# CEA-LIST/runia_core

Measured on AMD Instinct MI355X. Metric: OOD scores/sec, LaREM 16-MC PCA-256 (ResNet-18 layer4 latent 512x4x4), higher is better.
Workload: dtype f64

## Files before the change

### include/runia_hip.h

```cpp
#ifndef RUNIA_HIP_H
#define RUNIA_HIP_H

#include <stddef.h>
#include <stdint.h>

#ifdef __cplusplus
extern "C" {
#endif

#define RUNIA_OK 0
#define RUNIA_E_INVALID (-1)
#define RUNIA_E_LAUNCH (-2)
#define RUNIA_E_NODEVICE (-3)
#define RUNIA_E_WORKSPACE (-4)

typedef void* runia_stream_t;

int runia_abi_version(void);
const char* runia_error_string(int code);
int runia_device_count(void);
int runia_clock_probe(uint64_t* out4, int chain, runia_stream_t stream);
int runia_time_next_launch(void* start_event, void* stop_event);

int runia_mc_stack_f32(const float* x, const float* rand, int64_t rand_image_stride, float* out,
// ... 110 lines not shown
int runia_mc_entropy_f32(const float* x, const float* rand, int64_t rand_image_stride, double* h,
                         float* z_out, double* zero_fill, void* workspace, size_t workspace_bytes, int64_t N,
                         int C, int H, int W, int n_mc, double drop_prob, int block_size, int k, double min_dist,
                         runia_stream_t stream);
int runia_mc_draws_f32(float* out, int64_t N, int n_mc, int H, int W, uint64_t seed, int64_t first_image,
                       runia_stream_t stream);
int runia_mc_mask_table_counter_f32(uint64_t seed, int64_t first_image, void* workspace, size_t workspace_bytes,
                                    int64_t N, int H, int W, int n_mc, double drop_prob, int block_size,
                                    int redraw_dead_layers, runia_stream_t stream);
int runia_mc_entropy_counter_f32(const float* x, uint64_t seed, int64_t first_image, double* h, float* z_out,
                                 double* zero_fill, void* workspace, size_t workspace_bytes, int64_t N, int C, int H,
                                 int W, int n_mc, double drop_prob, int block_size, int k, double min_dist,
                                 int redraw_dead_layers, runia_stream_t stream);
int runia_pca_md_score_f64(const double* h, const double* packed_ct, const double* bias,
                           const double* scale, const double* md_mean, const double* packed_p,
                           double* score, double* y_out, int64_t N, int64_t D, int64_t n,
                           runia_stream_t stream);
size_t runia_proj_sq_workspace_bytes(int64_t N);
int runia_proj_sq_accumulate_f64(const double* h, const double* packed_m, const double* c, double* score,
                                 int64_t N, int64_t D, int64_t r, runia_stream_t stream);
int runia_proj_sq_score_f64(const double* h, const double* packed_m, const double* c, double* score,
                            void* workspace, size_t workspace_bytes, int64_t N, int64_t D, int64_t r,
                            runia_stream_t stream);

size_t runia_covariance_workspace_bytes(int64_t N, int64_t D);
int runia_covariance_f64(const double* x, double* mean, double* cov, void* workspace,
                         size_t workspace_bytes, int64_t N, int64_t D, runia_stream_t stream);
int runia_covariance_f32in(const float* x, double* mean, double* cov, void* workspace,
                           size_t workspace_bytes, int64_t N, int64_t D, runia_stream_t stream);

int runia_roi_align_f32(const float* input, const float* boxes, const int* batch_idx, float* out, int64_t K, int64_t B,
                        int C, int H, int W, int PH, int PW, double spatial_scale, int sampling_ratio, int aligned,
                        runia_stream_t stream);
int runia_nchw_to_nhwc_f32(const float* in, float* out, int64_t B, int C, int64_t HW, runia_stream_t stream);
int runia_roi_mc_entropy_supported(int PH, int PW, int n_mc, int k, int sampling_ratio);
size_t runia_roi_mc_entropy_workspace_bytes(int64_t K, int PH, int PW, int n_mc, int sampling_ratio);
int runia_roi_mc_entropy_f32(const float* feat_nhwc, const float* boxes, const int* batch_idx, const float* rand,
                             int64_t rand_image_stride, double* h, float* z_out, void* workspace, size_t workspace_bytes,
                             int64_t K, int64_t B, int C, int H, int W, int PH, int PW, double spatial_scale,
                             int sampling_ratio, int aligned, int n_mc, double drop_prob, int block_size, int k,
                             double min_dist, runia_stream_t stream);
#define RUNIA_ROI_MEANS_MAX_HW 2048
int runia_roi_means_f32(const float* feat_nhwc, const float* boxes, const int* batch_idx, float* out, int64_t ldo,
                        int64_t col_offset, int64_t K, int64_t B, int C, int H, int W, int PH, int PW, double spatial_scale,
                        int sampling_ratio, int aligned, runia_stream_t stream);

// ... 183 lines not shown
```

### runia_core_amd/_hip.py

```python
from __future__ import annotations

import contextlib
import ctypes
import os
import threading
from ctypes import c_char_p, c_double, c_float, c_int, c_int64, c_size_t, c_uint64, c_void_p
from typing import NamedTuple, Optional, Union

import numpy as np
import torch

from . import config as _config

_LIB_PATH = os.path.join(os.path.dirname(os.path.abspath(__file__)), "librunia_hip.so")
_lib: Optional[ctypes.CDLL] = None

_SIGNATURES = {
    "runia_abi_version": (c_int, []),
    "runia_error_string": (c_char_p, [c_int]),
    "runia_device_count": (c_int, []),
    "runia_clock_probe": (c_int, [c_void_p, c_int, c_void_p]),
    "runia_time_next_launch": (c_int, [c_void_p, c_void_p]),
    "runia_mc_stack_f32": (
        c_int,
        [c_void_p, c_void_p, c_int64, c_void_p, c_int64, c_int, c_int, c_int, c_int, c_double, c_int, c_void_p],
    ),
    "runia_mc_drop_flat_f32": (
        c_int,
        [c_void_p, c_void_p, c_int64, c_void_p, c_int64, c_int, c_int, c_int, c_int, c_double, c_int, c_void_p],
    ),
# ... 132 lines not shown
    "runia_roi_mc_entropy_supported": (c_int, [c_int, c_int, c_int, c_int, c_int]),
    "runia_roi_mc_entropy_workspace_bytes": (c_size_t, [c_int64, c_int, c_int, c_int, c_int]),
    "runia_roi_mc_entropy_f32": (
        c_int,
        [c_void_p, c_void_p, c_void_p, c_void_p, c_int64, c_void_p, c_void_p, c_void_p, c_size_t, c_int64, c_int64, c_int, c_int,
         c_int, c_int, c_int, c_double, c_int, c_int, c_int, c_double, c_int, c_int, c_double, c_void_p],
    ),
    "runia_roi_means_f32": (
        c_int,
        [c_void_p, c_void_p, c_void_p, c_void_p, c_int64, c_int64, c_int64, c_int64, c_int, c_int, c_int, c_int, c_int,
         c_double, c_int, c_int, c_void_p],
    ),
    "runia_linear_f32": (c_int, [c_void_p, c_void_p, c_void_p, c_void_p, c_int64, c_int64, c_int64, c_float, c_void_p]),
    "runia_ash_s_f32": (c_int, [c_void_p, c_void_p, c_int64, c_int64, c_int, c_void_p]),
    "runia_gen_score_f32": (c_int, [c_void_p, c_void_p, c_int64, c_int64, c_int, c_double, c_void_p]),
    "runia_gen_entropy_f32": (c_int, [c_void_p, c_void_p, c_int64, c_int64, c_int, c_double, c_void_p]),
    "runia_mcd_uncertainty_f32": (c_int, [c_void_p, c_void_p, c_void_p, c_void_p, c_int64, c_int, c_int64, c_void_p]),
    "runia_ash_s_rows_f32": (c_int, [c_void_p, c_void_p, c_void_p, c_int64, c_int64, c_int, c_int, c_void_p]),
    "runia_tril_inverse_f64": (c_int, [c_void_p, c_void_p, c_int64, c_int64, c_void_p]),
    "runia_proj_norm_f32": (c_int, [c_void_p, c_void_p, c_void_p, c_void_p, c_int64, c_int64, c_int64, c_void_p]),
    "runia_proj_norm_f64": (c_int, [c_void_p, c_void_p, c_void_p, c_void_p, c_int64, c_int64, c_int64, c_void_p]),
    "runia_proj_sq_workspace_bytes": (c_size_t, [c_int64]),
    "runia_proj_sq_accumulate_f64": (c_int, [c_void_p, c_void_p, c_void_p, c_void_p, c_int64, c_int64, c_int64, c_void_p]),
    "runia_proj_sq_score_f64": (
        c_int,
        [c_void_p, c_void_p, c_void_p, c_void_p, c_void_p, c_size_t, c_int64, c_int64, c_int64, c_void_p],
    ),
    "runia_covariance_workspace_bytes": (c_size_t, [c_int64, c_int64]),
    "runia_covariance_f64": (c_int, [c_void_p, c_void_p, c_void_p, c_void_p, c_size_t, c_int64, c_int64, c_void_p]),
    "runia_covariance_f32in": (c_int, [c_void_p, c_void_p, c_void_p, c_void_p, c_size_t, c_int64, c_int64, c_void_p]),
    "runia_rauq_workspace_bytes": (c_size_t, [c_int64, c_int64, c_int64, c_int64, c_int64, c_int]),
    "runia_rauq_gather": (c_int, [c_void_p, c_int, c_int64, c_int64, c_int64, c_int, c_void_p, c_void_p]),
    "runia_rauq_score": (
        c_int,
        [c_void_p, c_int64, c_int64, c_int64, c_int, c_void_p, c_void_p, c_int, c_void_p, c_void_p, c_void_p, c_size_t, c_void_p],
    ),
    "runia_rauq_rollout_rows": (
        c_int, [c_void_p, c_int, c_int64, c_int64, c_int64, c_int64, c_void_p, c_void_p, c_size_t, c_void_p]),
    "runia_rauq_rollout_att": (
        c_int,
        [c_void_p, c_int, c_int64, c_int64, c_int64, c_int64, c_int, c_int, c_int64, c_void_p, c_void_p, c_size_t, c_void_p],
    ),
    "runia_rauqb_workspace_bytes": (c_size_t, [c_int64, c_int64, c_int64, c_int64, c_int64, c_int]),
    "runia_rauqb_gather": (c_int, [c_void_p, c_void_p, c_int, c_int64, c_int64, c_int64, c_int64, c_int, c_void_p, c_void_p]),
    "runia_rauqb_score": (
        c_int,
        [c_void_p, c_void_p, c_int64, c_int64, c_int64, c_int64, c_int, c_int, c_void_p, c_int64, c_void_p, c_int, c_void_p,
# ... 918 lines not shown
        xp, hp = x.data_ptr() + done * c * hh * ww * 4, h.data_ptr() + done * c * 8
        rp = None if rand is None else rand.data_ptr() + done * stride * 4
        zp = None if z is None else z.data_ptr() + done * n_mc * c * 4
        zf = None if zero_fill is None else zero_fill.data_ptr() + done * 8
        if kernel_events is not None:
            if counter is not None:
                launch("runia_mc_mask_table_counter_f32", seed, int(counter.first_image) + done, ws.data_ptr(), ws_bytes, m, hh,
                       ww, n_mc, float(drop_prob), int(block_size), redraw)
            else:
                launch("runia_mc_mask_table_f32", rp, stride, ws.data_ptr(), ws_bytes, m, hh, ww, n_mc, float(drop_prob),
                       int(block_size))
            kernel_events.append(_timed_call("runia_mc_entropy_from_table_f32", xp, ws.data_ptr(), ws_bytes, hp, zp, zf, m, c, hh,
                                             ww, n_mc, int(k), float(min_dist)))
        elif counter is not None:
            launch("runia_mc_entropy_counter_f32", xp, seed, int(counter.first_image) + done, hp, zp, zf, ws.data_ptr(), ws_bytes,
                   m, c, hh, ww, n_mc, float(drop_prob), int(block_size), int(k), float(min_dist), redraw)
        else:
            launch("runia_mc_entropy_f32", xp, rp, stride, hp, zp, zf, ws.data_ptr(), ws_bytes, m, c, hh, ww, n_mc,
                   float(drop_prob), int(block_size), int(k), float(min_dist))
    return (h, z) if want_samples else h


@_device_guard()
def proj_sq_accumulate(h: torch.Tensor, packed_m: torch.Tensor, c: torch.Tensor, r: int, out: torch.Tensor) -> torch.Tensor:
    require_gpu()
    assert h.is_cuda and h.dtype == torch.float64 and h.dim() == 2
    h = h.contiguous()
    nrow, d = h.shape
    assert out.is_cuda and out.dtype == torch.float64 and out.shape == (nrow,) and out.is_contiguous()
    launch("runia_proj_sq_accumulate_f64", h.data_ptr(), packed_m.data_ptr(), c.data_ptr(), out.data_ptr(), nrow, d, int(r))
    return out


@_device_guard()
def pca_md_score(h: torch.Tensor, packed_ct: Optional[torch.Tensor], bias: Optional[torch.Tensor],
                 scale: Optional[torch.Tensor], md_mean: torch.Tensor, packed_p: torch.Tensor, n: int,
                 want_projection: bool = False, out: Optional[torch.Tensor] = None):
    require_gpu()
    assert h.is_cuda and h.dtype == torch.float64 and h.dim() == 2
    h = h.contiguous()
    nrow, d = h.shape
    if out is None:
        s = torch.empty((nrow,), dtype=torch.float64, device=h.device)
    else:
        assert out.is_cuda and out.dtype == torch.float64 and out.shape == (nrow,) and out.is_contiguous()
        s = out
    y = torch.empty((nrow, n), dtype=torch.float64, device=h.device) if want_projection else None
    launch("runia_pca_md_score_f64", h.data_ptr(), _ptr(packed_ct), _ptr(bias), _ptr(scale), md_mean.data_ptr(),
           packed_p.data_ptr(), s.data_ptr(), _ptr(y), nrow, d, n)
    return (s, y) if want_projection else s


@_device_guard()
# ... 133 lines not shown
@_device_guard()
def gen_score(logits: torch.Tensor, gamma: float, m: int) -> torch.Tensor:
    require_gpu()
    assert logits.is_cuda and logits.dtype == torch.float32 and logits.dim() == 2
    logits = logits.contiguous()
    s = torch.empty((logits.shape[0],), dtype=torch.float32, device=logits.device)
    launch("runia_gen_score_f32", logits.data_ptr(), s.data_ptr(), logits.shape[0], logits.shape[1], int(m), float(gamma))
    return s


@_device_guard()
def proj_norm(x: torch.Tensor, u: torch.Tensor, packed_ns: torch.Tensor, n: int) -> torch.Tensor:
    require_gpu()
    assert x.is_cuda and x.dim() == 2 and x.dtype == u.dtype and x.dtype in (torch.float32, torch.float64)
    x, u = x.contiguous(), u.contiguous()
    nrow, d = x.shape
    out = torch.empty((nrow,), dtype=torch.float64, device=x.device)
    launch("runia_proj_norm_f32" if x.dtype == torch.float32 else "runia_proj_norm_f64", x.data_ptr(), u.data_ptr(),
           packed_ns.data_ptr(), out.data_ptr(), nrow, d, int(n))
    return out


@_device_guard()
def proj_sq_score(h: torch.Tensor, packed_m: torch.Tensor, c: torch.Tensor, r: int, out: Optional[torch.Tensor] = None) -> torch.Tensor:
    lib = load_library()
    require_gpu()
    assert h.is_cuda and h.dtype == torch.float64 and h.dim() == 2
    h = h.contiguous()
    nrow, d = h.shape
    s = torch.empty((nrow,), dtype=torch.float64, device=h.device) if out is None else out
    ws_bytes = int(lib.runia_proj_sq_workspace_bytes(nrow))
    ws = torch.empty(max(ws_bytes, 16), dtype=torch.uint8, device=h.device)
    launch("runia_proj_sq_score_f64", h.data_ptr(), packed_m.data_ptr(), c.data_ptr(), s.data_ptr(), ws.data_ptr(), ws_bytes,
           nrow, d, int(r))
    return s


def _ood_metrics_buffers(n: int, device):
    ws_bytes = query("runia_ood_metrics_workspace_bytes", n)
    ws = workspace(ws_bytes + 256, device, 0)
    return ws, ws.data_ptr() + (-ws.data_ptr()) % 256, ws_bytes, torch.empty(3, dtype=torch.float64, device=device)


@_device_guard()
def ood_metrics(ind_scores: torch.Tensor, ood_scores: torch.Tensor) -> torch.Tensor:
    require_gpu()
    assert ind_scores.is_cuda and ood_scores.is_cuda and ind_scores.dtype == ood_scores.dtype
    assert ind_scores.dtype in (torch.float32, torch.float64)
    a, b = ind_scores.reshape(-1).contiguous(), ood_scores.reshape(-1).contiguous()
    n = a.numel() + b.numel()
    ws, ws_ptr, ws_bytes, out = _ood_metrics_buffers(n, a.device)
    launch("runia_ood_metrics_f64" if a.dtype == torch.float64 else "runia_ood_metrics_f32", a.data_ptr(), a.numel(),
           b.data_ptr(), b.numel(), out.data_ptr(), ws_ptr, ws_bytes)
    return out


@_device_guard()
def ood_clf_curve(ind_scores: torch.Tensor, ood_scores: torch.Tensor):
# ... 443 lines not shown
```

### runia_core_amd/csrc/fused.hip

```cpp
#include "common.hpp"
#include "entropy_core.hpp"
#include "mfma_f64_tile.hpp"
#include "philox.hpp"
#include "div_consts.hpp"

namespace {

using namespace runia_entropy;
using namespace runia_mfma;

constexpr int kMaxMC = 64;
typedef float f2 __attribute__((ext_vector_type(2)));

__device__ __forceinline__ void layer_consts(int cnt, int& m, float& flag, float& zh, float& zl) {
  const int a = cnt ? __ffs(cnt) - 1 : 0;
  m = cnt >> a;
  flag = __uint_as_float((unsigned)(127 - a) << 23);
  zh = cnt ? __uint_as_float(runia_div::kDivHi[(m - 1) >> 1]) : NAN;
  zl = cnt ? __uint_as_float(runia_div::kDivLo[(m - 1) >> 1]) : 0.f;
}

__device__ __forceinline__ float add_f32(float a, float b) {
  float r;
  asm("v_add_f32 %0, %1, %2" : "=v"(r) : "v"(a), "v"(b));
// ... 531 lines not shown
    const int64_t row = r0 + tid;
    if (row < g.N) g.score[row] = -(((part[tid] + part[BM + tid]) + part[2 * BM + tid]) + part[3 * BM + tid]);
  }
}

struct ProjSqArgs {
  const double* h;
  const double* packed_m;
  const double* c;
  double* score;
  double* partial;
  int64_t N, D, r;
};

#ifndef K2_WAVES
#define K2_WAVES 5
#endif
#ifndef K2_DMA
#define K2_DMA 1
#endif
#ifndef K2_WAVES_DMA
#define K2_WAVES_DMA 5
#endif
template <int RT, int NCT, bool ACCUMULATE, bool SPLIT, bool DMA>
__global__ __launch_bounds__(256, (RT == 1 && NCT <= 2) ? (DMA ? K2_WAVES_DMA : K2_WAVES) : 1) void proj_sq_kernel(ProjSqArgs g) {
#if defined(__HIP_DEVICE_COMPILE__)
  constexpr int BM = 16 * RT;
  __shared__ double lds_a[DMA ? 1 : 2 * BM * APITCH];
  __shared__ __attribute__((aligned(16))) double lds_d0[DMA ? BM * KC : 2];
  __shared__ __attribute__((aligned(16))) double lds_d1[DMA ? BM * KC : 2];
  constexpr int NG = (NCT + 1) / 2;
  __shared__ double part[4 * NG * BM];
  const int64_t n_pad = n_padded(g.r);
  const int tid = threadIdx.x, lane = tid & 63;
  const int wave = __builtin_amdgcn_readfirstlane(tid >> 6);
  const int li = lane & 15, lg = lane >> 4;
  const int64_t NT = n_pad / 16;
  int64_t tile = blockIdx.x;
  int half = 0;
  if constexpr (SPLIT) {
    tile = (int64_t)(blockIdx.x >> 4) * 8 + (blockIdx.x & 7);
    half = (blockIdx.x >> 3) & 1;
    if (tile * BM >= g.N) return;
  }
  const int64_t r0 = tile * BM;
  const int nchunks = (int)(k_padded(g.D) / KC);
  constexpr int PER_T = BM * KC / 256;
  double rowsq[NG][RT][4];
#pragma unroll
  for (int q = 0; q < NG; ++q)
#pragma unroll
    for (int a = 0; a < RT; ++a)
#pragma unroll
      for (int r = 0; r < 4; ++r) rowsq[q][a][r] = 0.0;
  for (int64_t cb = 0; cb < n_pad / BN; ++cb) {
    const int64_t ctbase = cb * 16 + (int64_t)half * (4 * NCT) + wave * NCT;
    d4 acc[RT][NCT];
#pragma unroll
    for (int a = 0; a < RT; ++a)
#pragma unroll
      for (int c = 0; c < NCT; ++c) acc[a][c] = (d4){0.0, 0.0, 0.0, 0.0};
    double2 bring[4][NCT];
    if constexpr (DMA) {
      const __amdgpu_buffer_rsrc_t brsrc = buffer_of(g.packed_m, (unsigned)(packed_elems(g.D, g.r) * 8));
      const int64_t rows_here = (g.N - r0 < BM) ? g.N - r0 : BM;
      const __amdgpu_buffer_rsrc_t arsrc = buffer_of(g.h + r0 * g.D, (unsigned)(rows_here * g.D * 8));
      const unsigned lane_bytes = (unsigned)lane * 16u;
      const unsigned pair_stride_bytes = (unsigned)NT * 1024u;
      const unsigned ct_bytes = (unsigned)ctbase * 1024u;
      constexpr int NDMA = BM / 4 / 4;
      unsigned a_lane_bytes[NDMA];
#pragma unroll
      for (int i = 0; i < NDMA; ++i) {
        const int slot = 64 * (wave + 4 * i) + lane;
        a_lane_bytes[i] = (unsigned)(((slot % BM) * g.D + 2 * (slot / BM)) * 8);
      }
      auto dma_rows = [&](int bufc, int kc) {
#pragma unroll
        for (int i = 0; i < NDMA; ++i)
          __builtin_amdgcn_raw_ptr_buffer_load_lds(
              arsrc, (__attribute__((address_space(3))) void*)((bufc ? lds_d1 : lds_d0) + 128 * (wave + 4 * i)), 16,
              a_lane_bytes[i], (unsigned)kc * 8u, 0, 0);
        asm volatile("" ::: "memory");
      };
      auto body = [&](auto buf_tag, int ch) {
        constexpr int bufc = decltype(buf_tag)::value;
        asm volatile("s_waitcnt vmcnt(%0)" ::"n"(3 * NCT) : "memory");
        __syncthreads();
        dma_rows(bufc ^ 1, ((ch + 1 < nchunks) ? ch + 1 : ch) * KC);
        mfma_chunk_dma<RT, NCT, BM>(acc, bufc ? lds_d1 : lds_d0, li, lg, brsrc, lane_bytes,
                                    ct_bytes + (unsigned)ch * 4u * pair_stride_bytes, pair_stride_bytes, bring);
      };
      dma_rows(0, 0);
#pragma unroll
      for (int j = 0; j < 3; ++j)
#pragma unroll
        for (int c = 0; c < NCT; ++c)
          bring[j][c] = __builtin_bit_cast(double2, __builtin_amdgcn_raw_buffer_load_b128(
                                                        brsrc, lane_bytes + c * 1024u, ct_bytes + j * pair_stride_bytes, 0));
      int ch = 0;
      for (; ch + 1 < nchunks; ch += 2) {
        body(std::integral_constant<int, 0>{}, ch);
        body(std::integral_constant<int, 1>{}, ch + 1);
      }
      if (ch < nchunks) body(std::integral_constant<int, 0>{}, ch);
    } else {
      const double2* bp = reinterpret_cast<const double2*>(g.packed_m) + ctbase * 64 + lane;
    #pragma unroll
      for (int j = 0; j < 3; ++j)
  #pragma unroll
        for (int c = 0; c < NCT; ++c) bring[j][c] = bp[j * NT * 64 + c * 64];
      double areg[PER_T];
      const int srow = tid / KC, skk = tid % KC;
      const bool interior = (r0 + BM <= g.N) && (g.D % KC == 0);
      const double* pa = g.h + (r0 + srow) * g.D + skk;
      auto load_a = [&](int64_t kc) {
        if (interior) {
  #pragma unroll
          for (int q = 0; q < PER_T; ++q) areg[q] = pa[(int64_t)q * (256 / KC) * g.D + kc];
          return;
        }
        const int64_t gk = kc + skk;
  #pragma unroll
        for (int q = 0; q < PER_T; ++q) {
          const int64_t gr = r0 + srow + q * (256 / KC);
          areg[q] = (gr < g.N && gk < g.D) ? g.h[gr * g.D + gk] : 0.0;
        }
      };
      load_a(0);
      int buf = 0;
      for (int64_t ch = 0; ch < nchunks; ++ch) {
  #pragma unroll
        for (int q = 0; q < PER_T; ++q) lds_a[(buf * BM + srow + q * (256 / KC)) * APITCH + skk] = areg[q];
        __syncthreads();
        if (ch + 1 < nchunks) load_a((ch + 1) * KC);
        mfma_chunk_ring<RT, NCT>(acc, lds_a + buf * BM * APITCH, APITCH, li, lg, bp + ch * 4 * NT * 64, NT * 64, bring);
        buf ^= 1;
      }
    }
#pragma unroll
    for (int a = 0; a < RT; ++a)
#pragma unroll
      for (int c = 0; c < NCT; ++c) {
        const int64_t col = (ctbase + c) * 16 + li;
        const double cc = (col < g.r) ? g.c[col] : 0.0;
#pragma unroll
        for (int r = 0; r < 4; ++r) {
          const double v = acc[a][c][r] + cc;
          rowsq[c / 2][a][r] = fma(v, v, rowsq[c / 2][a][r]);
        }
      }
    __syncthreads();
  }
#pragma unroll
  for (int q = 0; q < NG; ++q)
#pragma unroll
    for (int a = 0; a < RT; ++a)
#pragma unroll
      for (int r = 0; r < 4; ++r) {
        double v = rowsq[q][a][r];
        v += shfl_xor_f64(v, 1);
        v += shfl_xor_f64(v, 2);
        v += shfl_xor_f64(v, 4);
        v += shfl_xor_f64(v, 8);
        if (li == 0) part[(wave * NG + q) * BM + 16 * a + lg + 4 * r] = v;
      }
  __syncthreads();
  if (tid < BM) {
    const int64_t row = r0 + tid;
    if (row < g.N) {
      const double lo = ((part[tid] + part[BM + tid]) + part[2 * BM + tid]) + part[3 * BM + tid];
      if constexpr (NCT == 4) {
        const double hi = ((part[4 * BM + tid] + part[5 * BM + tid]) + part[6 * BM + tid]) + part[7 * BM + tid];
        g.score[row] = -(lo + hi);
      } else if constexpr (!SPLIT) {
        if constexpr (ACCUMULATE) unsafeAtomicAdd(&g.score[row], -lo);
        else g.score[row] = -lo;
      } else if constexpr (ACCUMULATE) {
        unsafeAtomicAdd(&g.score[row], -lo);
      } else {
        g.partial[(int64_t)half * g.N + row] = lo;
      }
    }
  }
#endif
}

__global__ void proj_sq_combine_kernel(const double* __restrict__ partial, double* __restrict__ score, int64_t N) {
// ... 287 lines not shown
  if (N == 0) return RUNIA_OK;
  if (!x || !h || N > 65535) return RUNIA_E_INVALID;
  if (!runia_mc_entropy_supported(H, W, n_mc, k)) return RUNIA_E_INVALID;
  if (!(((((uintptr_t)x) & 15) == 0) || (H * W) % 4 != 0)) return RUNIA_E_INVALID;
  if (int rc = runia_mc_mask_table_counter_f32(seed, first_image, workspace, workspace_bytes, N, H, W, n_mc,
                                               drop_prob, block_size, redraw_dead_layers, stream))
    return rc;
  return runia_mc_entropy_from_table_f32(x, workspace, workspace_bytes, h, z_out, zero_fill, N, C, H, W, n_mc, k,
                                         min_dist, stream);
}

extern "C" int runia_mc_entropy_supported(int H, int W, int n_mc, int k) {
  if (k != 5 || k >= n_mc) return 0;
  const bool hw = (H == 4 && W == 4);
  if (hw && n_mc > 4 && n_mc <= 32) return 1;
  if (n_mc > 8 && n_mc <= 32 && ((H == 2 && W == 2) || (H == 7 && W == 7) || (H == 8 && W == 8))) return 1;
  return 0;
}

static bool proj_sq_dma_ok(int64_t D, int64_t r) {
  return K2_DMA && D % KC == 0 && D < (1 << 23) && packed_elems(D, r) < ((int64_t)1 << 29);
}
static bool proj_sq_one_round(unsigned grid) { return (int64_t)grid <= (int64_t)K2_WAVES_DMA * runia_cu_count(); }
template <int RT, int NCT, bool ACCUMULATE, bool SPLIT>
static void launch_proj_sq(unsigned grid, hipStream_t s, const ProjSqArgs& g, bool dma) {
  if (dma && (RT > 1 || proj_sq_one_round(grid))) proj_sq_kernel<RT, NCT, ACCUMULATE, SPLIT, true><<<grid, 256, 0, s>>>(g);
  else proj_sq_kernel<RT, NCT, ACCUMULATE, SPLIT, false><<<grid, 256, 0, s>>>(g);
}

static bool proj_sq_large_tiles(int64_t N, int64_t cus) {
  const int64_t tiles32 = (N + 31) / 32;
  const int64_t rounds = (tiles32 + cus - 1) / cus;
  return tiles32 >= 2 * cus && 100 * tiles32 >= 93 * rounds * cus;
}

extern "C" int runia_proj_sq_accumulate_f64(const double* h, const double* packed_m, const double* c, double* score,
                                            int64_t N, int64_t D, int64_t r, runia_stream_t stream) {
  if (N < 0 || D <= 0 || r <= 0) return RUNIA_E_INVALID;
  if (N == 0) return RUNIA_OK;
  if (!h || !packed_m || !c || !score) return RUNIA_E_INVALID;
  ProjSqArgs g{h, packed_m, c, score, nullptr, N, D, r};
  hipStream_t s = as_stream(stream);
  const int64_t tiles16 = (N + 15) / 16, cus = runia_cu_count();
  const bool dma = proj_sq_dma_ok(D, r);
  if (r <= 64) launch_proj_sq<1, 1, true, false>((unsigned)tiles16, s, g, dma);
  else if (r <= 128) launch_proj_sq<1, 2, true, false>((unsigned)tiles16, s, g, dma);
  else if (proj_sq_large_tiles(N, cus)) launch_proj_sq<2, 4, false, false>((unsigned)((N + 31) / 32), s, g, dma);
  else if (tiles16 > cus / 2) launch_proj_sq<1, 2, true, true>((unsigned)((tiles16 + 7) / 8 * 16), s, g, dma);
  else launch_proj_sq<1, 4, false, false>((unsigned)tiles16, s, g, dma);
  return runia_check_launch();
}

extern "C" size_t runia_proj_sq_workspace_bytes(int64_t N) { return N > 0 ? (size_t)N * 2 * sizeof(double) : 0; }

extern "C" int runia_proj_sq_score_f64(const double* h, const double* packed_m, const double* c, double* score,
                                       void* workspace, size_t workspace_bytes, int64_t N, int64_t D, int64_t r,
                                       runia_stream_t stream) {
  if (N < 0 || D <= 0 || r <= 0) return RUNIA_E_INVALID;
  if (N == 0) return RUNIA_OK;
  if (!h || !packed_m || !c || !score) return RUNIA_E_INVALID;
  ProjSqArgs g{h, packed_m, c, score, reinterpret_cast<double*>(workspace), N, D, r};
  hipStream_t s = as_stream(stream);
  const int64_t tiles16 = (N + 15) / 16, cus = runia_cu_count();
  const bool dma = proj_sq_dma_ok(D, r);
  if (r <= 64) {
    launch_proj_sq<1, 1, false, false>((unsigned)tiles16, s, g, dma);
  } else if (r <= 128) {
    launch_proj_sq<1, 2, false, false>((unsigned)tiles16, s, g, dma);
  } else if (proj_sq_large_tiles(N, cus)) {
    launch_proj_sq<2, 4, false, false>((unsigned)((N + 31) / 32), s, g, dma);
  } else if (tiles16 > cus / 2 && workspace && workspace_bytes >= runia_proj_sq_workspace_bytes(N)) {
    launch_proj_sq<1, 2, false, true>((unsigned)((tiles16 + 7) / 8 * 16), s, g, dma);
    proj_sq_combine_kernel<<<(unsigned)((N + 255) / 256), 256, 0, s>>>(g.partial, score, N);
  } else {
    launch_proj_sq<1, 4, false, false>((unsigned)tiles16, s, g, dma);
  }
  return runia_check_launch();
}
```

### runia_core_amd/inference/pipeline.py

```python
from __future__ import annotations

from typing import Optional

import numpy as np
import torch
from torch import Tensor

from .. import _hip
from ..dimensionality_reduction import DevicePCA, device_pca_for
from ..evaluation.entropy import MIN_DIST, neighbors_for

__all__ = ["LaREMPipeline", "AsyncScores", "PreparedDraws"]


class PreparedDraws:

    def __init__(self, table: Tensor, ready: "torch.cuda.Event", slot: int, shape: tuple):
        self.table, self.ready, self.slot, self.shape = table, ready, slot, shape


class AsyncScores:

    def __init__(self, scores: Tensor, done: "torch.cuda.Event"):
        self.scores = scores
# ... 1 lines not shown

    def wait(self) -> Tensor:
        torch.cuda.current_stream().wait_event(self.done)
        return self.scores

    def result(self) -> np.ndarray:
        self.done.synchronize()
        return _hip.to_host(self.scores)


class LaREMPipeline:

    def __init__(self, postprocessor, pca_transform, mcd_samples_nro: int, drop_block_prob: float = 0.0,
                 drop_block_size: int = 1):
        self.postprocessor = postprocessor
        self.pca: Optional[DevicePCA] = device_pca_for(pca_transform) if pca_transform is not None else None
        self.n_mc = int(mcd_samples_nro)
        self.k = neighbors_for(self.n_mc)
        self.drop_prob = float(drop_block_prob)
        self.block_size = int(drop_block_size)
        self.overlap_chunks = 1
        self._side_streams = None
        self.fold_weights = True
        self._folded = None
        self._folded_fp = None
        self._k0 = None

    def prepare_draws(self, rand, n: int, h: int, w: int,
                      inputs_ready: Optional["torch.cuda.Event"] = None) -> Optional[PreparedDraws]:
        if not (0 < n <= 65535 and _hip.mc_entropy_supported(h, w, self.n_mc, self.k)):
            return None
        if self._k0 is None:
            self._k0 = {"stream": torch.cuda.Stream(), "tables": [None, None], "free": [None, None], "turn": 0}
        k0 = self._k0
        slot = k0["turn"]
        k0["turn"] ^= 1
        nbytes = max(16, int(_hip.load_library().runia_mc_entropy_workspace_bytes(n, h, w, self.n_mc)))
        if k0["tables"][slot] is None or k0["tables"][slot].numel() < nbytes:
            k0["tables"][slot] = torch.empty(nbytes, dtype=torch.uint8, device=_hip.require_gpu())
        s = k0["stream"]
        if inputs_ready is not None:
            s.wait_event(inputs_ready)
        elif not isinstance(rand, _hip.CounterDraws) and rand is not None:
            s.wait_stream(torch.cuda.current_stream())
        if k0["free"][slot] is not None:
            s.wait_event(k0["free"][slot])
# ... 20 lines not shown
                raise ValueError(f"prepared draws are for a batch of shape {prepared.shape}, got {(n, h, w)}")
            torch.cuda.current_stream().wait_event(prepared.ready)
            out = _hip.mc_entropy(latents, None, self.n_mc, self.drop_prob, self.block_size, self.k, MIN_DIST,
                                  kernel_events=kernel_events, zero_fill=zero_fill, table=prepared.table)
            self._k0["free"][prepared.slot] = torch.cuda.current_stream().record_event()
            return out
        if _hip.mc_entropy_supported(h, w, self.n_mc, self.k):
            return _hip.mc_entropy(latents, rand, self.n_mc, self.drop_prob if rand is not None else 0.0,
                                   self.block_size, self.k, MIN_DIST, kernel_events=kernel_events, zero_fill=zero_fill)
        if zero_fill is not None:
            zero_fill.zero_()
        return self.entropy(self.stack(latents, rand))

    def _md_state(self):
        pp = self.postprocessor
        if pp is None or not hasattr(pp, "_device_state") or not hasattr(pp, "feats_mean"):
            return None
        st = pp._device_state()
        return pp._mean(torch.float64), st["packed_p"]

    def _folded_state(self):
        pp = self.postprocessor
        fp = (_hip.array_fingerprint(pp.precision), _hip.array_fingerprint(pp.feats_mean),
              None if self.pca is None else id(self.pca))
        if self._folded is None or self._folded_fp != fp:
            self._folded_fp = fp
            prec = _hip.to_device(np.asarray(pp.precision, dtype=np.float64), torch.float64)
            lam, vec = _hip.eigh(prec)
            top = float(lam.abs().max()) if lam.numel() else 0.0
            if top == 0.0 or float(lam.min()) < -1e-10 * top:
                self._folded = False
                return None
            keep = lam > top * max(prec.shape) * np.finfo(np.float64).eps
            w = (torch.sqrt(lam[keep])[:, None] * vec[:, keep].t()).contiguous()
            mu = _hip.to_device(np.asarray(pp.feats_mean, dtype=np.float64).ravel(), torch.float64)
            if self.pca is not None:
                comp = _hip.to_device(self.pca.components_host, torch.float64)
                scale = self.pca.scale if self.pca.scale is not None else torch.ones_like(self.pca.bias)
                a = (comp / scale[:, None]).contiguous()
                b = -self.pca.bias / scale - mu
                m = _hip.matmul_f64(w, a)
            else:
                b = -mu
                m = w
            c = _hip.matmul_f64(w, b.reshape(-1, 1).contiguous()).reshape(-1).contiguous()
            self._folded = (_hip.pack_weights(m.t().contiguous()), c, int(m.shape[0]))
        return self._folded or None

    def score_entropies(self, h: Tensor) -> Tensor:
        md = self._md_state()
        if md is not None and h.dtype == torch.float64:
            mean, packed_p = md
            if self.pca is not None and h.shape[1] != self.pca.n_features:
                raise ValueError(f"X has {h.shape[1]} features, but PCA is expecting {self.pca.n_features} features as input.")
            if self.fold_weights:
                folded = self._folded_state()
                if folded is not None:
                    return _hip.proj_sq_score(h, *folded)
            if self.pca is not None:
                if h.shape[1] != self.pca.n_features:
                    raise ValueError(f"X has {h.shape[1]} features, but PCA is expecting {self.pca.n_features} features as input.")
                return _hip.pca_md_score(h, self.pca.packed_ct, self.pca.bias, self.pca.scale, mean, packed_p,
                                         self.pca.n_components)
            return _hip.pca_md_score(h, None, None, None, mean, packed_p, h.shape[1])
        y = self.pca.transform_device(h) if self.pca is not None else h
        return self.postprocessor.postprocess_device(y)

    def _score_h_into(self, h: Tensor, out: Tensor, mean: Tensor, packed_p: Tensor) -> None:
        folded = self._folded_state() if self.fold_weights else None
        if folded is not None:
            _hip.proj_sq_score(h, *folded, out=out)
        elif self.pca is not None:
            _hip.pca_md_score(h, self.pca.packed_ct, self.pca.bias, self.pca.scale, mean, packed_p,
                              self.pca.n_components, out=out)
        else:
            _hip.pca_md_score(h, None, None, None, mean, packed_p, h.shape[1], out=out)

    def score_samples(self, z: Tensor) -> Tensor:
        return self.score_entropies(self.entropy(z))

    def score_latents(self, latents: Tensor, rand, chunks: Optional[int] = None,
                      k1_events: Optional[list] = None, prepared: Optional[PreparedDraws] = None) -> Tensor:
        n, _, hh, ww = latents.shape
        chunks = self.overlap_chunks if chunks is None else int(chunks)
        md = self._md_state()
        fused = _hip.mc_entropy_supported(hh, ww, self.n_mc, self.k) and md is not None
        counter = isinstance(rand, _hip.CounterDraws)
        if prepared is not None and not fused:
            prepared = None
        if prepared is not None or not fused or chunks <= 1 or n < 2048 * chunks or (rand is not None and not counter and rand.dim() != 4):
            folded = self._folded_state() if (fused and self.fold_weights) else None
            if folded is not None and (self.pca is None or latents.shape[1] == self.pca.n_features):
                scores = torch.empty((n,), dtype=torch.float64, device=latents.device)
                h = self.entropy_from_latents(latents, rand, k1_events, zero_fill=scores, prepared=prepared)
                return _hip.proj_sq_accumulate(h, *folded, out=scores)
            return self.score_entropies(self.entropy_from_latents(latents, rand, k1_events if fused else None,
                                                                  prepared=prepared))
        latents = latents.contiguous()
        if rand is not None and not counter:
            rand = rand.contiguous()
        mean, packed_p = md
        main = torch.cuda.current_stream()
        if self._side_streams is None:
            self._side_streams = (torch.cuda.Stream(), torch.cuda.Stream())
        s_k1, s_k2 = self._side_streams
        h = torch.empty((n, latents.shape[1]), dtype=torch.float64, device=latents.device)
        scores = torch.empty((n,), dtype=torch.float64, device=latents.device)
        start = main.record_event()
        s_k1.wait_event(start)
        s_k2.wait_event(start)
        per = -(-n // chunks)
        drop = self.drop_prob if rand is not None else 0.0
        for a in range(0, n, per):
            b = min(a + per, n)
            with torch.cuda.stream(s_k1):
                r_ab = None if rand is None else (rand._replace(first_image=rand.first_image + a) if counter else rand[a:b])
                _hip.mc_entropy(latents[a:b], r_ab, self.n_mc, drop, self.block_size,
                                self.k, MIN_DIST, out=h[a:b], kernel_events=k1_events)
# ... 57 lines not shown
```

Baseline: 57.67 million.

## QR-fold projection to upper trapezoid and skip zero K-chunks in proj_sq kernel

```diff
diff --git a/include/runia_hip.h b/include/runia_hip.h
--- a/include/runia_hip.h
+++ b/include/runia_hip.h
@@ -156,6 +156,13 @@
 int runia_proj_sq_score_f64(const double* h, const double* packed_m, const double* c, double* score,
                             void* workspace, size_t workspace_bytes, int64_t N, int64_t D, int64_t r,
                             runia_stream_t stream);
+int runia_proj_sq_accumulate_trap_f64(const double* h, const double* packed_m, const double* c, double* score,
+                                      int64_t N, int64_t D, int64_t r, runia_stream_t stream);
+int runia_proj_sq_score_trap_f64(const double* h, const double* packed_m, const double* c, double* score,
+                                 void* workspace, size_t workspace_bytes, int64_t N, int64_t D, int64_t r,
+                                 runia_stream_t stream);
+int runia_qr_trapezoid_f64(const double* m, const double* c, double* r_out, double* c_out, int64_t r, int64_t D,
+                           runia_stream_t stream);
 
 size_t runia_covariance_workspace_bytes(int64_t N, int64_t D);
 int runia_covariance_f64(const double* x, double* mean, double* cov, void* workspace,
diff --git a/runia_core_amd/_hip.py b/runia_core_amd/_hip.py
--- a/runia_core_amd/_hip.py
+++ b/runia_core_amd/_hip.py
@@ -5,7 +5,7 @@
 import os
 import threading
 from ctypes import c_char_p, c_double, c_float, c_int, c_int64, c_size_t, c_uint64, c_void_p
-from typing import NamedTuple, Optional, Union
+from typing import NamedTuple, Optional, Tuple, Union
 
 import numpy as np
 import torch
@@ -184,7 +184,13 @@
     "runia_proj_norm_f64": (c_int, [c_void_p, c_void_p, c_void_p, c_void_p, c_int64, c_int64, c_int64, c_void_p]),
     "runia_proj_sq_workspace_bytes": (c_size_t, [c_int64]),
     "runia_proj_sq_accumulate_f64": (c_int, [c_void_p, c_void_p, c_void_p, c_void_p, c_int64, c_int64, c_int64, c_void_p]),
+    "runia_proj_sq_accumulate_trap_f64": (c_int, [c_void_p, c_void_p, c_void_p, c_void_p, c_int64, c_int64, c_int64, c_void_p]),
+    "runia_qr_trapezoid_f64": (c_int, [c_void_p, c_void_p, c_void_p, c_void_p, c_int64, c_int64, c_void_p]),
     "runia_proj_sq_score_f64": (
+        c_int,
+        [c_void_p, c_void_p, c_void_p, c_void_p, c_void_p, c_size_t, c_int64, c_int64, c_int64, c_void_p],
+    ),
+    "runia_proj_sq_score_trap_f64": (
         c_int,
         [c_void_p, c_void_p, c_void_p, c_void_p, c_void_p, c_size_t, c_int64, c_int64, c_int64, c_void_p],
     ),
@@ -1149,13 +1155,15 @@
 
 
 @_device_guard()
-def proj_sq_accumulate(h: torch.Tensor, packed_m: torch.Tensor, c: torch.Tensor, r: int, out: torch.Tensor) -> torch.Tensor:
+def proj_sq_accumulate(h: torch.Tensor, packed_m: torch.Tensor, c: torch.Tensor, r: int, out: torch.Tensor,
+                       trap: bool = False) -> torch.Tensor:
     require_gpu()
     assert h.is_cuda and h.dtype == torch.float64 and h.dim() == 2
     h = h.contiguous()
     nrow, d = h.shape
     assert out.is_cuda and out.dtype == torch.float64 and out.shape == (nrow,) and out.is_contiguous()
-    launch("runia_proj_sq_accumulate_f64", h.data_ptr(), packed_m.data_ptr(), c.data_ptr(), out.data_ptr(), nrow, d, int(r))
+    launch("runia_proj_sq_accumulate_trap_f64" if trap else "runia_proj_sq_accumulate_f64", h.data_ptr(), packed_m.data_ptr(),
+           c.data_ptr(), out.data_ptr(), nrow, d, int(r))
     return out
 
 
@@ -1335,7 +1343,8 @@
 
 
 @_device_guard()
-def proj_sq_score(h: torch.Tensor, packed_m: torch.Tensor, c: torch.Tensor, r: int, out: Optional[torch.Tensor] = None) -> torch.Tensor:
+def proj_sq_score(h: torch.Tensor, packed_m: torch.Tensor, c: torch.Tensor, r: int, out: Optional[torch.Tensor] = None,
+                  trap: bool = False) -> torch.Tensor:
     lib = load_library()
     require_gpu()
     assert h.is_cuda and h.dtype == torch.float64 and h.dim() == 2
@@ -1344,9 +1353,20 @@
     s = torch.empty((nrow,), dtype=torch.float64, device=h.device) if out is None else out
     ws_bytes = int(lib.runia_proj_sq_workspace_bytes(nrow))
     ws = torch.empty(max(ws_bytes, 16), dtype=torch.uint8, device=h.device)
-    launch("runia_proj_sq_score_f64", h.data_ptr(), packed_m.data_ptr(), c.data_ptr(), s.data_ptr(), ws.data_ptr(), ws_bytes,
-           nrow, d, int(r))
+    launch("runia_proj_sq_score_trap_f64" if trap else "runia_proj_sq_score_f64", h.data_ptr(), packed_m.data_ptr(),
+           c.data_ptr(), s.data_ptr(), ws.data_ptr(), ws_bytes, nrow, d, int(r))
     return s
+
+
+@_device_guard()
+def qr_trapezoid(m: torch.Tensor, c: torch.Tensor) -> Tuple[torch.Tensor, torch.Tensor]:
+    require_gpu()
+    assert m.is_cuda and m.dtype == torch.float64 and m.dim() == 2 and m.shape[0] <= m.shape[1]
+    assert c.is_cuda and c.dtype == torch.float64 and c.shape == (m.shape[0],)
+    m, c = m.contiguous(), c.contiguous()
+    r_out, c_out = torch.empty_like(m), torch.empty_like(c)
+    launch("runia_qr_trapezoid_f64", m.data_ptr(), c.data_ptr(), r_out.data_ptr(), c_out.data_ptr(), m.shape[0], m.shape[1])
+    return r_out, c_out
 
 
 def _ood_metrics_buffers(n: int, device):
diff --git a/runia_core_amd/csrc/fused.hip b/runia_core_amd/csrc/fused.hip
--- a/runia_core_amd/csrc/fused.hip
+++ b/runia_core_amd/csrc/fused.hip
@@ -577,10 +577,17 @@
 #ifndef K2_WAVES_DMA
 #define K2_WAVES_DMA 5
 #endif
-template <int RT, int NCT, bool ACCUMULATE, bool SPLIT, bool DMA>
+#ifndef K2_TRAP_FORM
+#define K2_TRAP_FORM 2
+#endif
+#ifndef K2_TRAP_ROT
+#define K2_TRAP_ROT 2
+#endif
+template <int RT, int NCT, bool ACCUMULATE, bool SPLIT, bool DMA, int TRAP = 0>
 __global__ __launch_bounds__(256, (RT == 1 && NCT <= 2) ? (DMA ? K2_WAVES_DMA : K2_WAVES) : 1) void proj_sq_kernel(ProjSqArgs g) {
 #if defined(__HIP_DEVICE_COMPILE__)
   constexpr int BM = 16 * RT;
+  constexpr bool WAVE_SKIP = TRAP == 2 && DMA && RT == 1;
   __shared__ double lds_a[DMA ? 1 : 2 * BM * APITCH];
   __shared__ __attribute__((aligned(16))) double lds_d0[DMA ? BM * KC : 2];
   __shared__ __attribute__((aligned(16))) double lds_d1[DMA ? BM * KC : 2];
@@ -600,6 +607,10 @@
   }
   const int64_t r0 = tile * BM;
   const int nchunks = (int)(k_padded(g.D) / KC);
+  const int rot = K2_TRAP_ROT == 1 ? (int)(tile & 3)
+                  : K2_TRAP_ROT == 2 ? (int)(((blockIdx.x >> 4) + (blockIdx.x >> 8)) & 3)
+                  : K2_TRAP_ROT == 3 ? (int)((blockIdx.x >> 8) & 3) : 0;
+  const int grp = WAVE_SKIP ? (wave + rot) & 3 : wave;
   constexpr int PER_T = BM * KC / 256;
   double rowsq[NG][RT][4];
 #pragma unroll
@@ -609,7 +620,10 @@
 #pragma unroll
       for (int r = 0; r < 4; ++r) rowsq[q][a][r] = 0.0;
   for (int64_t cb = 0; cb < n_pad / BN; ++cb) {
-    const int64_t ctbase = cb * 16 + (int64_t)half * (4 * NCT) + wave * NCT;
+    const int64_t ctbase = cb * 16 + (int64_t)half * (4 * NCT) + grp * NCT;
+    const int64_t wg_chunk = (cb * 16 + (int64_t)half * (4 * NCT)) * 16 / KC, wave_chunk = ctbase * 16 / KC;
+    const int ch0 = TRAP ? (int)(wg_chunk < nchunks - 1 ? wg_chunk : nchunks - 1) : 0;
+    [[maybe_unused]] const int ws = WAVE_SKIP ? (int)(wave_chunk < nchunks - 1 ? wave_chunk : nchunks - 1) : ch0;
     d4 acc[RT][NCT];
 #pragma unroll
     for (int a = 0; a < RT; ++a)
@@ -646,21 +660,35 @@
         mfma_chunk_dma<RT, NCT, BM>(acc, bufc ? lds_d1 : lds_d0, li, lg, brsrc, lane_bytes,
                                     ct_bytes + (unsigned)ch * 4u * pair_stride_bytes, pair_stride_bytes, bring);
       };
-      dma_rows(0, 0);
+      dma_rows(0, ch0 * KC);
+      int ch = ch0;
+      if constexpr (WAVE_SKIP) {
+        for (; ch < ws; ++ch) {
+          asm volatile("s_waitcnt vmcnt(0)" ::: "memory");
+          __syncthreads();
+          dma_rows((ch + 1 - ch0) & 1, (ch + 1) * KC);
+        }
+      }
 #pragma unroll
       for (int j = 0; j < 3; ++j)
 #pragma unroll
         for (int c = 0; c < NCT; ++c)
           bring[j][c] = __builtin_bit_cast(double2, __builtin_amdgcn_raw_buffer_load_b128(
-                                                        brsrc, lane_bytes + c * 1024u, ct_bytes + j * pair_stride_bytes, 0));
-      int ch = 0;
+                                                        brsrc, lane_bytes + c * 1024u,
+                                                        ct_bytes + (unsigned)(4 * ch + j) * pair_stride_bytes, 0));
+      if constexpr (WAVE_SKIP) {
+        if ((ch - ch0) & 1) {
+          body(std::integral_constant<int, 1>{}, ch);
+          ++ch;
+        }
+      }
       for (; ch + 1 < nchunks; ch += 2) {
         body(std::integral_constant<int, 0>{}, ch);
         body(std::integral_constant<int, 1>{}, ch + 1);
       }
       if (ch < nchunks) body(std::integral_constant<int, 0>{}, ch);
     } else {
-      const double2* bp = reinterpret_cast<const double2*>(g.packed_m) + ctbase * 64 + lane;
+      const double2* bp = reinterpret_cast<const double2*>(g.packed_m) + ctbase * 64 + lane + (int64_t)ch0 * 4 * NT * 64;
     #pragma unroll
       for (int j = 0; j < 3; ++j)
   #pragma unroll
@@ -682,14 +710,14 @@
           areg[q] = (gr < g.N && gk < g.D) ? g.h[gr * g.D + gk] : 0.0;
         }
       };
-      load_a(0);
+      load_a((int64_t)ch0 * KC);
       int buf = 0;
-      for (int64_t ch = 0; ch < nchunks; ++ch) {
+      for (int64_t ch = ch0; ch < nchunks; ++ch) {
   #pragma unroll
         for (int q = 0; q < PER_T; ++q) lds_a[(buf * BM + srow + q * (256 / KC)) * APITCH + skk] = areg[q];
         __syncthreads();
         if (ch + 1 < nchunks) load_a((ch + 1) * KC);
-        mfma_chunk_ring<RT, NCT>(acc, lds_a + buf * BM * APITCH, APITCH, li, lg, bp + ch * 4 * NT * 64, NT * 64, bring);
+        mfma_chunk_ring<RT, NCT>(acc, lds_a + buf * BM * APITCH, APITCH, li, lg, bp + (ch - ch0) * 4 * NT * 64, NT * 64, bring);
         buf ^= 1;
       }
     }
@@ -718,7 +746,7 @@
         v += shfl_xor_f64(v, 2);
         v += shfl_xor_f64(v, 4);
         v += shfl_xor_f64(v, 8);
-        if (li == 0) part[(wave * NG + q) * BM + 16 * a + lg + 4 * r] = v;
+        if (li == 0) part[(grp * NG + q) * BM + 16 * a + lg + 4 * r] = v;
       }
   __syncthreads();
   if (tid < BM) {
@@ -1052,10 +1080,17 @@
   return K2_DMA && D % KC == 0 && D < (1 << 23) && packed_elems(D, r) < ((int64_t)1 << 29);
 }
 static bool proj_sq_one_round(unsigned grid) { return (int64_t)grid <= (int64_t)K2_WAVES_DMA * runia_cu_count(); }
-template <int RT, int NCT, bool ACCUMULATE, bool SPLIT>
+template <bool TRAP, int RT, int NCT, bool ACCUMULATE, bool SPLIT>
 static void launch_proj_sq(unsigned grid, hipStream_t s, const ProjSqArgs& g, bool dma) {
-  if (dma && (RT > 1 || proj_sq_one_round(grid))) proj_sq_kernel<RT, NCT, ACCUMULATE, SPLIT, true><<<grid, 256, 0, s>>>(g);
-  else proj_sq_kernel<RT, NCT, ACCUMULATE, SPLIT, false><<<grid, 256, 0, s>>>(g);
+  const bool use_dma = dma && (RT > 1 || proj_sq_one_round(grid));
+  if constexpr (TRAP) {
+    if (use_dma) proj_sq_kernel<RT, NCT, ACCUMULATE, SPLIT, true, K2_TRAP_FORM><<<grid, 256, 0, s>>>(g);
+    else if constexpr (RT > 1) proj_sq_kernel<RT, NCT, ACCUMULATE, SPLIT, false, K2_TRAP_FORM><<<grid, 256, 0, s>>>(g);
+    else proj_sq_kernel<RT, NCT, ACCUMULATE, SPLIT, false><<<grid, 256, 0, s>>>(g);
+  } else {
+    if (use_dma) proj_sq_kernel<RT, NCT, ACCUMULATE, SPLIT, true><<<grid, 256, 0, s>>>(g);
+    else proj_sq_kernel<RT, NCT, ACCUMULATE, SPLIT, false><<<grid, 256, 0, s>>>(g);
+  }
 }
 
 static bool proj_sq_large_tiles(int64_t N, int64_t cus) {
@@ -1064,8 +1099,9 @@
   return tiles32 >= 2 * cus && 100 * tiles32 >= 93 * rounds * cus;
 }
 
-extern "C" int runia_proj_sq_accumulate_f64(const double* h, const double* packed_m, const double* c, double* score,
-                                            int64_t N, int64_t D, int64_t r, runia_stream_t stream) {
+template <bool TRAP>
+static int proj_sq_accumulate(const double* h, const double* packed_m, const double* c, double* score, int64_t N, int64_t D,
+                              int64_t r, runia_stream_t stream) {
   if (N < 0 || D <= 0 || r <= 0) return RUNIA_E_INVALID;
   if (N == 0) return RUNIA_OK;
   if (!h || !packed_m || !c || !score) return RUNIA_E_INVALID;
@@ -1073,19 +1109,29 @@
   hipStream_t s = as_stream(stream);
   const int64_t tiles16 = (N + 15) / 16, cus = runia_cu_count();
   const bool dma = proj_sq_dma_ok(D, r);
-  if (r <= 64) launch_proj_sq<1, 1, true, false>((unsigned)tiles16, s, g, dma);
-  else if (r <= 128) launch_proj_sq<1, 2, true, false>((unsigned)tiles16, s, g, dma);
-  else if (proj_sq_large_tiles(N, cus)) launch_proj_sq<2, 4, false, false>((unsigned)((N + 31) / 32), s, g, dma);
-  else if (tiles16 > cus / 2) launch_proj_sq<1, 2, true, true>((unsigned)((tiles16 + 7) / 8 * 16), s, g, dma);
-  else launch_proj_sq<1, 4, false, false>((unsigned)tiles16, s, g, dma);
+  if (r <= 64) launch_proj_sq<TRAP, 1, 1, true, false>((unsigned)tiles16, s, g, dma);
+  else if (r <= 128) launch_proj_sq<TRAP, 1, 2, true, false>((unsigned)tiles16, s, g, dma);
+  else if (proj_sq_large_tiles(N, cus)) launch_proj_sq<TRAP, 2, 4, false, false>((unsigned)((N + 31) / 32), s, g, dma);
+  else if (tiles16 > cus / 2) launch_proj_sq<TRAP, 1, 2, true, true>((unsigned)((tiles16 + 7) / 8 * 16), s, g, dma);
+  else launch_proj_sq<TRAP, 1, 4, false, false>((unsigned)tiles16, s, g, dma);
   return runia_check_launch();
 }
 
+extern "C" int runia_proj_sq_accumulate_f64(const double* h, const double* packed_m, const double* c, double* score,
+                                            int64_t N, int64_t D, int64_t r, runia_stream_t stream) {
+  return proj_sq_accumulate<false>(h, packed_m, c, score, N, D, r, stream);
+}
+extern "C" int runia_proj_sq_accumulate_trap_f64(const double* h, const double* packed_m, const double* c, double* score,
+                                                 int64_t N, int64_t D, int64_t r, runia_stream_t stream) {
+  if (r > D) return RUNIA_E_INVALID;
+  return proj_sq_accumulate<true>(h, packed_m, c, score, N, D, r, stream);
+}
+
 extern "C" size_t runia_proj_sq_workspace_bytes(int64_t N) { return N > 0 ? (size_t)N * 2 * sizeof(double) : 0; }
 
-extern "C" int runia_proj_sq_score_f64(const double* h, const double* packed_m, const double* c, double* score,
-                                       void* workspace, size_t workspace_bytes, int64_t N, int64_t D, int64_t r,
-                                       runia_stream_t stream) {
+template <bool TRAP>
+static int proj_sq_score(const double* h, const double* packed_m, const double* c, double* score, void* workspace,
+                         size_t workspace_bytes, int64_t N, int64_t D, int64_t r, runia_stream_t stream) {
   if (N < 0 || D <= 0 || r <= 0) return RUNIA_E_INVALID;
   if (N == 0) return RUNIA_OK;
   if (!h || !packed_m || !c || !score) return RUNIA_E_INVALID;
@@ -1094,16 +1140,28 @@
   const int64_t tiles16 = (N + 15) / 16, cus = runia_cu_count();
   const bool dma = proj_sq_dma_ok(D, r);
   if (r <= 64) {
-    launch_proj_sq<1, 1, false, false>((unsigned)tiles16, s, g, dma);
+    launch_proj_sq<TRAP, 1, 1, false, false>((unsigned)tiles16, s, g, dma);
   } else if (r <= 128) {
-    launch_proj_sq<1, 2, false, false>((unsigned)tiles16, s, g, dma);
+    launch_proj_sq<TRAP, 1, 2, false, false>((unsigned)tiles16, s, g, dma);
   } else if (proj_sq_large_tiles(N, cus)) {
-    launch_proj_sq<2, 4, false, false>((unsigned)((N + 31) / 32), s, g, dma);
+    launch_proj_sq<TRAP, 2, 4, false, false>((unsigned)((N + 31) / 32), s, g, dma);
   } else if (tiles16 > cus / 2 && workspace && workspace_bytes >= runia_proj_sq_workspace_bytes(N)) {
-    launch_proj_sq<1, 2, false, true>((unsigned)((tiles16 + 7) / 8 * 16), s, g, dma);
+    launch_proj_sq<TRAP, 1, 2, false, true>((unsigned)((tiles16 + 7) / 8 * 16), s, g, dma);
     proj_sq_combine_kernel<<<(unsigned)((N + 255) / 256), 256, 0, s>>>(g.partial, score, N);
   } else {
-    launch_proj_sq<1, 4, false, false>((unsigned)tiles16, s, g, dma);
+    launch_proj_sq<TRAP, 1, 4, false, false>((unsigned)tiles16, s, g, dma);
   }
   return runia_check_launch();
 }
+
+extern "C" int runia_proj_sq_score_f64(const double* h, const double* packed_m, const double* c, double* score,
+                                       void* workspace, size_t workspace_bytes, int64_t N, int64_t D, int64_t r,
+                                       runia_stream_t stream) {
+  return proj_sq_score<false>(h, packed_m, c, score, workspace, workspace_bytes, N, D, r, stream);
+}
+extern "C" int runia_proj_sq_score_trap_f64(const double* h, const double* packed_m, const double* c, double* score,
+                                            void* workspace, size_t workspace_bytes, int64_t N, int64_t D, int64_t r,
+                                            runia_stream_t stream) {
+  if (r > D) return RUNIA_E_INVALID;
+  return proj_sq_score<true>(h, packed_m, c, score, workspace, workspace_bytes, N, D, r, stream);
+}
diff --git a/runia_core_amd/csrc/qr.hip b/runia_core_amd/csrc/qr.hip
--- /dev/null
+++ b/runia_core_amd/csrc/qr.hip
@@ -0,0 +1,86 @@
+#include "common.hpp"
+
+namespace {
+
+constexpr int kQrThreads = 1024, kQrLanes = 512, kQrSlices = kQrThreads / kQrLanes;
+constexpr int64_t kQrMaxRows = 4096;
+
+__global__ __launch_bounds__(kQrThreads) void qr_trapezoid_kernel(const double* __restrict__ m, const double* __restrict__ c,
+                                                                   double* __restrict__ a, double* __restrict__ q, int64_t r,
+                                                                   int64_t D) {
+  __shared__ double v[kQrMaxRows];
+  __shared__ double ps[kQrSlices][kQrLanes];
+  __shared__ double scal[2];
+  const int tid = threadIdx.x, lane = tid & 63;
+  const int cl = tid % kQrLanes, sl = tid / kQrLanes;
+  if (a != m)
+    for (int64_t e = tid; e < r * D; e += kQrThreads) a[e] = m[e];
+  if (q != c)
+    for (int64_t e = tid; e < r; e += kQrThreads) q[e] = c[e];
+  __syncthreads();
+  for (int64_t j = 0; j + 1 < r; ++j) {
+    const int64_t rows = r - j;
+    for (int64_t i = tid; i < rows; i += kQrThreads) v[i] = a[(j + i) * D + j];
+    __syncthreads();
+    if (tid < 64) {
+      double s = 0.0;
+      for (int64_t i = 1 + lane; i < rows; i += 64) s = fma(v[i], v[i], s);
+      s += shfl_xor_f64(s, 1);
+      s += shfl_xor_f64(s, 2);
+      s += shfl_xor_f64(s, 4);
+      s += shfl_xor_f64(s, 8);
+      s += shfl_xor_f64(s, 16);
+      s += shfl_xor_f64(s, 32);
+      if (lane == 0) {
+        const double x0 = v[0];
+        if (s == 0.0) {
+          scal[0] = x0;
+          scal[1] = 0.0;
+        } else {
+          const double norm = sqrt(fma(x0, x0, s));
+          const double alpha = (x0 > 0.0) ? -norm : norm;
+          v[0] = x0 - alpha;
+          scal[0] = alpha;
+          scal[1] = norm * (norm + fabs(x0));
+        }
+      }
+    }
+    __syncthreads();
+    const double alpha = scal[0], denom = scal[1];
+    if (denom != 0.0) {
+      const int64_t half = (rows + 1) / 2;
+      const int64_t i0 = sl * half, i1 = (i0 + half < rows) ? i0 + half : rows;
+      for (int64_t kb = j + 1; kb <= D; kb += kQrLanes) {
+        const int64_t k = kb + cl;
+        const bool live = k <= D;
+        double* col = (k < D) ? a + j * D + k : q + j;
+        const int64_t stride = (k < D) ? D : 1;
+        double s = 0.0;
+        if (live) {
+#pragma unroll 8
+          for (int64_t i = i0; i < i1; ++i) s = fma(v[i], col[i * stride], s);
+        }
+        ps[sl][cl] = s;
+        __syncthreads();
+        if (live) {
+          const double w = (ps[0][cl] + ps[1][cl]) / denom;
+#pragma unroll 8
+          for (int64_t i = i0; i < i1; ++i) col[i * stride] = fma(-v[i], w, col[i * stride]);
+        }
+        __syncthreads();
+      }
+    }
+    for (int64_t i = tid; i < rows; i += kQrThreads) a[(j + i) * D + j] = (i == 0) ? alpha : 0.0;
+    __syncthreads();
+  }
+}
+
+}
+
+extern "C" int runia_qr_trapezoid_f64(const double* m, const double* c, double* r_out, double* c_out, int64_t r, int64_t D,
+                                      runia_stream_t stream) {
+  if (r <= 0 || D <= 0 || r > D || r > kQrMaxRows) return RUNIA_E_INVALID;
+  if (!m || !c || !r_out || !c_out) return RUNIA_E_INVALID;
+  qr_trapezoid_kernel<<<1, kQrThreads, 0, as_stream(stream)>>>(m, c, r_out, c_out, r, D);
+  return runia_check_launch();
+}
diff --git a/runia_core_amd/inference/pipeline.py b/runia_core_amd/inference/pipeline.py
--- a/runia_core_amd/inference/pipeline.py
+++ b/runia_core_amd/inference/pipeline.py
@@ -47,6 +47,7 @@
         self.overlap_chunks = 1
         self._side_streams = None
         self.fold_weights = True
+        self.fold_trapezoid = True
         self._folded = None
         self._folded_fp = None
         self._k0 = None
@@ -113,7 +114,7 @@
     def _folded_state(self):
         pp = self.postprocessor
         fp = (_hip.array_fingerprint(pp.precision), _hip.array_fingerprint(pp.feats_mean),
-              None if self.pca is None else id(self.pca))
+              None if self.pca is None else id(self.pca), bool(self.fold_trapezoid))
         if self._folded is None or self._folded_fp != fp:
             self._folded_fp = fp
             prec = _hip.to_device(np.asarray(pp.precision, dtype=np.float64), torch.float64)
@@ -135,7 +136,10 @@
                 b = -mu
                 m = w
             c = _hip.matmul_f64(w, b.reshape(-1, 1).contiguous()).reshape(-1).contiguous()
-            self._folded = (_hip.pack_weights(m.t().contiguous()), c, int(m.shape[0]))
+            trap = bool(self.fold_trapezoid) and m.shape[0] <= m.shape[1]
+            if trap:
+                m, c = _hip.qr_trapezoid(m.contiguous(), c)
+            self._folded = (_hip.pack_weights(m.t().contiguous()), c, int(m.shape[0]), trap)
         return self._folded or None
 
     def score_entropies(self, h: Tensor) -> Tensor:
@@ -147,7 +151,7 @@
             if self.fold_weights:
                 folded = self._folded_state()
                 if folded is not None:
-                    return _hip.proj_sq_score(h, *folded)
+                    return _hip.proj_sq_score(h, *folded[:3], trap=folded[3])
             if self.pca is not None:
                 if h.shape[1] != self.pca.n_features:
                     raise ValueError(f"X has {h.shape[1]} features, but PCA is expecting {self.pca.n_features} features as input.")
@@ -160,7 +164,7 @@
     def _score_h_into(self, h: Tensor, out: Tensor, mean: Tensor, packed_p: Tensor) -> None:
         folded = self._folded_state() if self.fold_weights else None
         if folded is not None:
-            _hip.proj_sq_score(h, *folded, out=out)
+            _hip.proj_sq_score(h, *folded[:3], out=out, trap=folded[3])
         elif self.pca is not None:
             _hip.pca_md_score(h, self.pca.packed_ct, self.pca.bias, self.pca.scale, mean, packed_p,
                               self.pca.n_components, out=out)
@@ -184,7 +188,7 @@
             if folded is not None and (self.pca is None or latents.shape[1] == self.pca.n_features):
                 scores = torch.empty((n,), dtype=torch.float64, device=latents.device)
                 h = self.entropy_from_latents(latents, rand, k1_events, zero_fill=scores, prepared=prepared)
-                return _hip.proj_sq_accumulate(h, *folded, out=scores)
+                return _hip.proj_sq_accumulate(h, *folded[:3], out=scores, trap=folded[3])
             return self.score_entropies(self.entropy_from_latents(latents, rand, k1_events if fused else None,
                                                                   prepared=prepared))
         latents = latents.contiguous()
```

After: 59.82 million (median of 6 runs). +3.7%, better.
